# isl-org/Open3D-PointNet2-Semantic3D

Measured on AMD Instinct MI355X. Metric: points/sec through SA+FP stack (B=16,N=8192), higher is better.
Workload: dtype f32

## Files before the change

benchlib/accounting.py:

```python
import json
import os

import torch

ROOT = os.path.dirname(os.path.dirname(os.path.abspath(__file__)))

HBM_PEAK_GBS = 8000.0
MFMA_F32_PEAK_TF = 157.3

FPS_KERNELS = ("farthest_point_sample", "fps_gather", "fps_nested")
LATENCY_KERNELS = FPS_KERNELS + ("coarse_geometry", "ball_query_bin")

PMC_FILE = "profiles/r06_pmc_hbm_traffic.json"
PMC_KERNEL_OF = {"fp_mlp_fused_pre": "fp_chain_pipe_kernel", "fp_mlp_fused": "sa_fused_kernel<2", "sa_mlp_max_fused": "sa_fused_kernel<3, 1, 1, 2"}


def pmc_traffic(kernel):
    try:
        with open(os.path.join(ROOT, PMC_FILE)) as f:
            ks = json.load(f)["kernels"]
    except (OSError, ValueError, KeyError):
        return None
    key = PMC_KERNEL_OF.get(kernel, kernel)
    hits = [v["traffic_bytes"] for k, v in ks.items() if key in k]
# ... 18 lines not shown
        b, n, m, _, ns = a[:5]
        return "hbm", b * n * 12 + b * m * 12 + b * m * ns * 4 + b * m * 4
    if name == "pn2_ball_query_bin":
        b, n = a[:2]
        return "hbm", b * n * 12 + b * n * 14
    if name == "pn2_group_point":
        b, n, c, m, ns = a[:5]
        return "hbm", b * m * ns * 4 + b * n * c * 4 + b * m * ns * c * 4
    if name == "pn2_sa_group_concat":
        b, n, m, ns, c = a[:5]
        return "hbm", b * m * ns * 4 + b * n * (3 + c) * 4 + b * m * 12 + b * m * ns * (3 + c) * 4
    if name == "pn2_three_nn":
        b, n, m = a[:3]
        return "hbm", b * n * 12 + b * m * 12 + b * n * 24
    if name == "pn2_three_interpolate":
        b, m, c, n = a[:4]
        return "hbm", b * m * c * 4 + b * n * 24 + b * n * c * 4
    if name == "pn2_fp_interp_concat":
        b, n, m, c1, c2 = a[:5]
        return "hbm", b * m * c2 * 4 + b * n * 24 + b * n * c1 * 4 + b * n * (c1 + c2) * 4
    if name == "pn2_linear":
        rows, cin, cout = a[:3]
        return "mfma", 2 * rows * cin * cout
    if name == "pn2_mlp_chain":
        rows, cin, L = a[0], a[1], a[2]
        widths = a[4:4 + L]
        fl = 0
        for w in widths:
            fl += 2 * rows * cin * w
            cin = w
        return "mfma", fl
    if name == "pn2_mlp_wide":
        rows, cin, L = a[0], a[1], a[3]
        fl = 0
        for w in a[6:6 + L]:
            fl += 2 * rows * cin * w
            cin = w
        return "mfma", fl
    if name == "pn2_sa_mlp_wide":
        b, n, m, ns, c, L = a[:6]
        cin, fl = 3 + c, 0
        for w in a[7:7 + L]:
            fl += 2 * b * m * ns * cin * w
            cin = w
        return "mfma", fl
    if name == "pn2_fp_mlp_wide":
# ... 117 lines not shown
```

include/pn2_abi.h:

```cpp
#ifndef PN2_ABI_H_
#define PN2_ABI_H_

#include <stddef.h>
#include <stdint.h>

#ifdef __cplusplus
extern "C" {
#endif

#define PN2_ABI_VERSION 2

#define PN2_OK 0
#define PN2_EINVAL (-1)
#define PN2_ENULL (-2)
#define PN2_ERANGE (-3)
#define PN2_EUNSUP (-4)

#define PN2_ARITH_STRICT 0
#define PN2_ARITH_FMA 1
#define PN2_ARITH_FMA_ALT 2

int pn2_abi_version(void);
const char *pn2_build_info(void);
const char *pn2_strerror(int code);
// ... 217 lines not shown
                       const double *scene_z_size, const float *label_weights, int num_label_weights, double half_x,
                       double half_y, unsigned long long seed, long long *counter, const int *draw_scene,
                       const int *draw_center, const unsigned char *draw_mask, int mask_cap, const double *draw_rot,
                       void *workspace, size_t workspace_bytes, int *out_info, double *out_finfo, int *out_sel,
                       float *out_data, int *out_labels, float *out_weights, void *stream);

int pn2_scene_ingest_workspace_size(int n, unsigned long long *bytes);
int pn2_scene_ingest(int n, const double *points, const double *colors, const int *labels, double *out_points,
                     float *out_colors, unsigned char *out_labels, int *out_perm, double *out_zrange, long long *out_hist,
                     int *status, void *workspace, size_t workspace_bytes, void *stream);

int pn2_fp_mlp_fused_pre(int b, int n, int m, int c1, const float *dist, const int *idx, const float *points1,
                         const float *z, int nlayers, const int *widths, const float *const *w,
                         const float *const *bias, float *y, void *stream);
int pn2_fp_mlp_fused_pre_ld(int b, int n, int m, int c1, const float *dist, const int *idx, const float *points1,
                            int ld_points1, const float *z, int nlayers, const int *widths, const float *const *w,
                            const float *const *bias, float *y, void *stream);

int pn2_fp_mlp_fused_pre_schedule(int b, int n, int m, int c1, const float *dist, const int *idx, const float *points1,
                                  const float *z, int nlayers, const int *widths, const float *const *w,
                                  const float *const *bias, float *y, int schedule, void *stream);

int pn2_set_sa_row_packing(int on);

int pn2_sa_mlp_fused_pre(int b, int n, int m, int nsample, const float *xyz, const float *new_xyz, const float *zf,
                         const int *idx, int nlayers, const int *widths, const float *const *w,
                         const float *const *bias, int pool, float *out, void *stream);

int pn2_fp_mlp_wide_pre(int b, int n, int m, int c1, const float *dist, const int *idx, const float *points1,
                        const float *z, int nlayers, const int *widths, const float *const *w,
                        const float *const *bias, float *y, void *stream);
int pn2_sa_mlp_wide_pre(int b, int n, int m, int nsample, const float *xyz, const float *new_xyz, const float *zf,
                        const int *idx, int nlayers, const int *widths, const float *const *w,
                        const float *const *bias, int pool, float *y, void *stream);

size_t pn2_ball_query_bin_bytes(int n);
int pn2_ball_query_bin(int b, int n, float radius, const float *xyz1, void *workspace, size_t workspace_bytes, void *stream);
int pn2_ball_query_bin_ld(int b, int n, float radius, const float *xyz1, int ld1, void *workspace, size_t workspace_bytes,
                          void *stream);
int pn2_query_ball_point_binned(int b, int n, int m, float radius, int nsample, const float *xyz1, const float *xyz2,
                                const void *bins, int *idx, int *pts_cnt, int arith_mode, void *stream);

int pn2_group_pool(long long rows, int k, int c, int mode, const float *x, const float *gxyz, float *out, void *stream);
int pn2_group_pool_grad(long long rows, int k, int c, int mode, const float *x, const float *gxyz, const float *dout,
                        float *dx, void *stream);

// ... 225 lines not shown
```

open3d-pointnet2-semantic3d_amd/csrc/pn2_linear.hip:

```cpp
#include <type_traits>

#include "pn2_common.h"
#include "pn2_mfma_stats.h"
#include "pn2_fwd_narrow.h"
#include "pn2_dgrad_wide.h"

namespace {

template <int U, int N, class F>
__device__ __forceinline__ void static_for(F& f) {
    if constexpr (U < N) {
        f(std::integral_constant<int, U>{});
        static_for<U + 1, N>(f);
    }
}

constexpr int kBK = 32;
constexpr int kAS = kBK + 4;

__device__ __forceinline__ void atomic_max_nonneg(float* addr, float v) {
    atomicMax(reinterpret_cast<int*>(addr), __float_as_int(v));
}

template <int WM, int WN, int NT, bool VEC_A, int WK = 1, int ST = 2, bool TB = false, bool XF = false, int GX = 0>
__global__ void __launch_bounds__(256)
linear_kernel(int rows, int cin, int cout, const float* __restrict__ x,
              const float* __restrict__ w, const float* __restrict__ bias, int relu, int pool,
              float* __restrict__ y, double* __restrict__ stats = nullptr, Pn2BnGradEpilogue gepi = Pn2BnGradEpilogue{},
// ... 625 lines not shown
                v = fmaxf(v, __shfl_xor(v, 32));
                v += bb;
                if (relu) v = fmaxf(v, 0.f);
                if (half == 0 && wrow0 < rows) y[(size_t)(wrow0 / 32) * cout + col] = v;
            }
        }
    }
    }
    pn2_bn_finish(fin, gridDim.x * gridDim.y, blockIdx.x + gridDim.x * blockIdx.y);
}

template <int TM, int TN, int G = 2>
int launch_linear_splitk(int rows, int cin, int cout, const float* x, const float* w, const float* bias, int relu,
                         int pool, float* y, hipStream_t st, double* stats = nullptr, const Pn2BnFinish* fin = nullptr) {
    dim3 grid((rows + 32 * TM - 1) / (32 * TM), cout / (32 * TN));
    const bool vec_a = (cin % 4 == 0) && ((uintptr_t)x % 16 == 0);
    const Pn2BnFinish f = fin ? *fin : Pn2BnFinish{};
    if (vec_a) linear_splitk_kernel<TM, TN, true, G><<<grid, 256, 0, st>>>(rows, cin, cout, x, w, bias, relu, pool, y, stats, f);
    else linear_splitk_kernel<TM, TN, false, G><<<grid, 256, 0, st>>>(rows, cin, cout, x, w, bias, relu, pool, y, stats, f);
    PN2_RETURN_IF_LAUNCH_FAILED();
    return PN2_OK;
}

template <int TM, int TN, bool XF = false, int GX = 0, int NWV = 4>
__global__ void __launch_bounds__(64 * NWV, NWV == 4 ? 2 : 1)
linear_wgrad_kernel(int rows, int cin, int cout, int chunk, const float* __restrict__ x,
                    const float* __restrict__ dy, float* __restrict__ dw, Pn2LoadTransform xf = Pn2LoadTransform{},
                    Pn2GradOnLoad gx = Pn2GradOnLoad{}) {
    const int lane = threadIdx.x & 63, half = lane >> 5, l31 = lane & 31;
    const int wave = __builtin_amdgcn_readfirstlane(threadIdx.x >> 6);
    const long long c0 = ((long long)blockIdx.x * NWV + wave) * chunk;
    const int r0 = c0 < rows ? (int)c0 : rows;
    const int r1 = c0 + chunk < rows ? (int)(c0 + chunk) : rows;
    const int m0 = blockIdx.y * 32 * TM, n0 = blockIdx.z * 32 * TN;
    const int hoff = rows > 1 ? half : 0;
    unsigned offa[TM], offb[TN];
#pragma unroll
    for (int t = 0; t < TM; ++t) { const int m = m0 + t * 32 + l31; offa[t] = (unsigned)(hoff * cin + (m < cin ? m : cin - 1)); }
#pragma unroll
    for (int t = 0; t < TN; ++t) { const int n = n0 + t * 32 + l31; offb[t] = (unsigned)(hoff * cout + (n < cout ? n : cout - 1)); }
    float xsc[TM], xsh[TM];
#pragma unroll
    for (int t = 0; t < TM; ++t) {
        const int m = m0 + t * 32 + l31;
        xsc[t] = XF ? xf.scale[m < cin ? m : cin - 1] : 1.f;
        xsh[t] = XF ? xf.shift[m < cin ? m : cin - 1] : 0.f;
// ... 206 lines not shown
    if (cout % 128 == 0 && g_lin_cfg != 0 && g_lin_cfg < 5) {
        if (g_lin_cfg == 1) return PN2_LIN(4, 1, 4, 1);
        if (g_lin_cfg == 2) return PN2_LIN(2, 2, 2, 1);
        if (g_lin_cfg == 3) return PN2_LIN(1, 4, 1, 1);
        return PN2_LIN(1, 2, 1, 2);
    }
    if (cout % 128 == 0) {
        const long long cb = cout / 128;
        const bool vec_a = (cin % 4 == 0) && ((uintptr_t)x % 16 == 0);
        if (((rows + 127) / 128) * cb >= 512 && vec_a && cb > 1) return PN2_LIN(4, 1, 4, 1);
        if (((rows + 63) / 64) * cb >= 512) return PN2_LIN(2, 2, 2, 1);
        if (((rows + 31) / 32) * cb >= 256 || cin < 128) return PN2_LIN(1, 4, 1, 1);
        return PN2_LIN(1, 2, 1, 2);
    }
    if (cout % 64 == 0 && pool <= 1 && rows <= 32768) return PN2_LIN(1, 2, 1, 2);
    if (cout % 64 == 0) return PN2_LIN(4, 1, 2, 1);
    return PN2_LIN(4, 1, 1, 1);
#undef PN2_LIN
}

extern "C" int pn2_linear(int rows, int cin, int cout, const float* x, const float* w,
                          const float* bias, int relu, int pool, float* y, void* stream) {
    return linear_impl(rows, cin, cout, x, w, bias, relu, pool, y, stream, nullptr);
}

extern "C" int pn2_linear_narrow(int rows, int cin, int cout, const float* x, const float* w, const float* bias, float* y,
                                 void* stream) {
    if (rows <= 0 || cin <= 0 || cout <= 0) return PN2_EINVAL;
    if (!x || !w || !y) return PN2_ENULL;
    if (cout > 16 || cin % 4 != 0 || ((uintptr_t)x % 16) != 0 || (size_t)cin * cout * sizeof(float) > 48 * 1024) return PN2_EUNSUP;
    if ((long long)rows + 128 > 0x7fffffffLL) return PN2_ERANGE;
    hipStream_t st = static_cast<hipStream_t>(stream);
    switch (cout) {
#define PN2_NW(N_) case N_: return launch_linear_narrow<N_>(rows, cin, x, w, bias, y, st);
        PN2_NW(1) PN2_NW(2) PN2_NW(3) PN2_NW(4) PN2_NW(5) PN2_NW(6) PN2_NW(7) PN2_NW(8) PN2_NW(9) PN2_NW(10) PN2_NW(11)
        PN2_NW(12) PN2_NW(13) PN2_NW(14) PN2_NW(15) PN2_NW(16)
#undef PN2_NW
    }
    return PN2_EUNSUP;
}

extern "C" int pn2_linear_bn_stats(int rows, int cin, int cout, const float* x, const float* w, float* y,
                                   void* bn_workspace, size_t workspace_bytes, void* stream) {
    if (!bn_workspace) return PN2_ENULL;
    if (!pn2_bn_ws_fits(bn_workspace, workspace_bytes, cout)) return PN2_EINVAL;
    return linear_impl(rows, cin, cout, x, w, nullptr, 0, 0, y, stream, static_cast<double*>(bn_workspace));
// ... 277 lines not shown
```

open3d-pointnet2-semantic3d_amd/csrc/pn2_sa_fused.hip:

```cpp
#include "pn2_common.h"
#include "pn2_layer_stack.h"
#include <atomic>
#include <type_traits>
#include <utility>

namespace {

typedef float f32x4 __attribute__((ext_vector_type(4)));
typedef float f32x16 __attribute__((ext_vector_type(16)));

struct SaFusedParams {
    int n, m, c, groups;
    int kshift;
    int rows;
    int w[3];
    const float* xyz;
    const float* new_xyz;
    const float* points;
    const int* idx;
    const float* dist;
    const float* points1;
    int c1;
    int ldx, ldp, ld1;
    const float* W[3];
// ... 158 lines not shown
        if (kshift == 4) {
            float v0 = acc[nt][0], v1 = acc[nt][8];
#pragma unroll
            for (int r = 1; r < 8; ++r) { v0 = fmaxf(v0, acc[nt][r]); v1 = fmaxf(v1, acc[nt][8 + r]); }
            v0 = fmaxf(v0, __shfl_xor(v0, 32));
            v1 = fmaxf(v1, __shfl_xor(v1, 32));
            if (half == 0) {
                out[(size_t)(2 * g) * wout + nt * 32 + l31] = fmaxf(v0 + bv, 0.f);
                out[(size_t)(2 * g + 1) * wout + nt * 32 + l31] = fmaxf(v1 + bv, 0.f);
            }
        } else {
            float v = acc[nt][0];
#pragma unroll
            for (int r = 1; r < 16; ++r) v = fmaxf(v, acc[nt][r]);
            v = fmaxf(v, __shfl_xor(v, 32));
            v = fmaxf(v + bv, 0.f);
            if (half == 0)
                atomicMax(reinterpret_cast<int*>(out + (size_t)(g >> (kshift - 5)) * wout + nt * 32 + l31), __float_as_int(v));
        }
    }
}

template <int NT>
__device__ __forceinline__ void pool_store_packed(const f32x16 (&acc)[NT], const float* __restrict__ sbias, float* __restrict__ out,
                                                  int wout, int sshift, int nvalid, const int (&gq)[4], int half, int l31) {
#pragma unroll
    for (int nt = 0; nt < NT; ++nt) {
        const float bv = sbias[nt * 32 + l31];
        float v[4];
#pragma unroll
        for (int q = 0; q < 4; ++q)
            v[q] = fmaxf(fmaxf(acc[nt][4 * q], acc[nt][4 * q + 1]), fmaxf(acc[nt][4 * q + 2], acc[nt][4 * q + 3]));
        if (sshift == 3) {
#pragma unroll
            for (int q = 0; q < 4; ++q) {
                const float u = fmaxf(v[q], __shfl_xor(v[q], 32));
                if (half == 0 && q < nvalid) out[(size_t)gq[q] * wout + nt * 32 + l31] = fmaxf(u + bv, 0.f);
            }
        } else if (sshift == 4) {
#pragma unroll
            for (int q = 0; q < 2; ++q) {
                float u = fmaxf(v[2 * q], v[2 * q + 1]);
                u = fmaxf(u, __shfl_xor(u, 32));
                if (half == 0 && q < nvalid) out[(size_t)gq[q] * wout + nt * 32 + l31] = fmaxf(u + bv, 0.f);
            }
        } else {
            float u = fmaxf(fmaxf(v[0], v[1]), fmaxf(v[2], v[3]));
            u = fmaxf(u, __shfl_xor(u, 32));
            if (half == 0) out[(size_t)gq[0] * wout + nt * 32 + l31] = fmaxf(u + bv, 0.f);
        }
    }
}

template <int NT>
__device__ __forceinline__ void rows_store(const f32x16 (&acc)[NT], const float* __restrict__ sbias,
                                           float* __restrict__ obase, int wout, int row0, int rows,
                                           int half, int l31) {
    if (row0 + 32 <= rows) {
        float* __restrict__ o = obase + (size_t)(row0 + 4 * half) * wout + l31;
#pragma unroll
        for (int nt = 0; nt < NT; ++nt) {
            const float bv = sbias[nt * 32 + l31];
#pragma unroll
            for (int r = 0; r < 16; ++r)
                o[((r & 3) + 8 * (r >> 2)) * wout + nt * 32] = fmaxf(acc[nt][r] + bv, 0.f);
        }
        return;
    }
#pragma unroll
    for (int nt = 0; nt < NT; ++nt) {
        const float bv = sbias[nt * 32 + l31];
#pragma unroll
        for (int r = 0; r < 16; ++r) {
            const int row = row0 + acc_chan(r, half);
            if (row < rows) obase[(size_t)row * wout + nt * 32 + l31] = fmaxf(acc[nt][r] + bv, 0.f);
        }
    }
// ... 109 lines not shown
        stage1(sb3, W3, p.bias[2]);
    }
    __syncthreads();
    PN2_CHAIN_STAMP(1);

    constexpr int WOUT = L == 1 ? W1 : (L == 2 ? W2 : W3);
    int g_lo = blockIdx.x * NW + wave, g_hi = p.groups, g_step = gridDim.x * NW;
    if ((gridDim.x & 7u) == 0u && (p.groups & 7) == 0) {
        const int per = p.groups >> 3, xcd = blockIdx.x & 7, slot = blockIdx.x >> 3;
        g_lo = xcd * per + slot * NW + wave;
        g_hi = (xcd + 1) * per;
        g_step = (gridDim.x >> 3) * NW;
    }
    int pk_b = 0, pk_nb = 0, pk_bstep = 1, pk_lo = 0, pk_hi = 0;
    if constexpr (PACK) {
        pk_lo = 0; pk_hi = p.groups; pk_b = blockIdx.x; pk_bstep = gridDim.x;
        if ((gridDim.x & 7u) == 0u && (p.groups & 7) == 0) {
            const int per = p.groups >> 3, xcd = blockIdx.x & 7;
            pk_lo = xcd * per; pk_hi = pk_lo + per; pk_b = blockIdx.x >> 3; pk_bstep = gridDim.x >> 3;
        }
        pk_nb = (pk_hi - pk_lo + p.blk - 1) / p.blk;
    }
    for (bool pk_first = true;; pk_b += pk_bstep, pk_first = false) {
    int pk_base = 0, pk_n32 = 0, pk_t16 = 0, pk_n16 = 0, pk_n8 = 0;
    if constexpr (PACK) {
        if (pk_b >= pk_nb) break;
        if (!pk_first) __syncthreads();
        pk_base = pk_lo + pk_b * p.blk;
        const int cnt = min(p.blk, pk_hi - pk_base);
        for (int c0 = 2 * wave; c0 < cnt; c0 += 2 * NW) {
            const int cl = c0 + half;
            const int v = p.idx[(size_t)(pk_base + (cl < cnt ? cl : c0)) * 32 + l31];
            const int first = __shfl(v, lane & 32);
            const unsigned long long diff = __ballot(v != first);
            const unsigned mine = (unsigned)(diff >> (lane & 32));
            const int live = 32 - __clz(mine | 1u);
            if (l31 == 0 && cl < cnt) s_cls[cl] = live <= 8 ? 8 : (live <= 16 ? 16 : 32);
        }
        __syncthreads();
        const int cls = lane < cnt ? s_cls[lane] : 0;
        const unsigned long long m32 = __ballot(cls == 32), m16 = __ballot(cls == 16), m8 = __ballot(cls == 8);
        const int n16 = __popcll(m16), n8 = __popcll(m8);
        const int promote = ((n16 & 1) && (n8 & 3) == 1) ? 1 : 0;
        pk_n32 = __popcll(m32); pk_n16 = n16 + promote; pk_n8 = n8 - promote;
        pk_t16 = (pk_n16 + 1) >> 1;
        if (wave == 0 && lane < cnt) {
            const unsigned long long below = (1ull << lane) - 1ull;
            int tile, slot;
            if (cls == 32) { tile = __popcll(m32 & below); slot = 0; }
            else {
                int c = cls, r = __popcll((cls == 16 ? m16 : m8) & below);
                if (promote && c == 8 && r == n8 - 1) { c = 16; r = n16; }
                if (c == 16) { tile = pk_n32 + (r >> 1); slot = r & 1; }
                else { tile = pk_n32 + pk_t16 + (r >> 2); slot = r & 3; }
            }
            s_desc[tile * 4 + slot] = pk_base + lane;
        }
        __syncthreads();
        g_lo = wave; g_hi = pk_n32 + pk_t16 + ((pk_n8 + 3) >> 2); g_step = NW;
    }
    for (int g = g_lo; g < g_hi; g += g_step, ++tile_no) {
        PN2_CHAIN_STAMP(2);
        size_t prow;
        int pk_sshift = 5, pk_nvalid = 1, pk_gq[4] = {0, 0, 0, 0};
        (void)pk_sshift; (void)pk_nvalid; (void)pk_gq;
        f32x16 a1[NT1];
        zero_acc<NT1>(a1);
        constexpr bool LAST1 = (L == 1);
        const float* w1l = wp1 + half * W1 + l31 * NT1;
        constexpr int S0 = DENSE ? 0 : 2;
        if constexpr (DENSE) {
            const int row = g * 32 + l31;
            prow = (size_t)(row < p.rows ? row : p.rows - 1);
        } else {
            int grp, ii;
            if constexpr (PACK) {
                if (g < pk_n32) { pk_sshift = 5; pk_nvalid = 1; }
                else if (g < pk_n32 + pk_t16) { pk_sshift = 4; pk_nvalid = min(2, pk_n16 - 2 * (g - pk_n32)); }
                else { pk_sshift = 3; pk_nvalid = min(4, pk_n8 - 4 * (g - pk_n32 - pk_t16)); }
#pragma unroll
                for (int q = 0; q < 4; ++q) pk_gq[q] = __builtin_amdgcn_readfirstlane(s_desc[g * 4 + (q < pk_nvalid ? q : 0)]);
                const int q = l31 >> pk_sshift;
                grp = q == 1 ? pk_gq[1] : (q == 2 ? pk_gq[2] : (q == 3 ? pk_gq[3] : pk_gq[0]));
                ii = p.idx[(size_t)grp * 32 + (l31 & ((1 << pk_sshift) - 1))];
            } else {
                grp = (g * 32 + l31) >> p.kshift;
                ii = p.idx[(size_t)g * 32 + l31];
            }
            const int bi = grp / p.m;
            prow = (size_t)bi * p.n + ii;
            const float cxv = p.new_xyz[(size_t)grp * 3 + 0];
            const float cyv = p.new_xyz[(size_t)grp * 3 + 1];
            const float czv = p.new_xyz[(size_t)grp * 3 + 2];
            const float rx = p.xyz[prow * p.ldx + 0] - cxv;
            const float ry = p.xyz[prow * p.ldx + 1] - cyv;
            const float rz = p.xyz[prow * p.ldx + 2] - czv;
            mfma_step<NT1, LAST1>(a1, w1l + 0 * 2 * W1, half ? ry : rx);
            mfma_step<NT1, LAST1>(a1, w1l + 1 * 2 * W1, half ? 0.f : rz);
        }
        if constexpr (INTERP) {
            const float* __restrict__ dr = p.dist + prow * 3;
            const int* __restrict__ ir = p.idx + prow * 3;
            const float d1 = fmaxf(dr[0], 1e-10f), d2 = fmaxf(dr[1], 1e-10f), d3 = fmaxf(dr[2], 1e-10f);
            const float r1 = 1.0f / d1, r2 = 1.0f / d2, r3 = 1.0f / d3;
// ... 407 lines not shown
        p.stats[256 + 2048 + blockIdx.x * NW + wave] = (long long)__builtin_amdgcn_s_memrealtime();
        p.stats[256 + 3072 + blockIdx.x * NW + wave] = t_real0;
    }
    if (p.trace && lane == 0) {
        const int wv = blockIdx.x * NW + wave;
        unsigned long long* cnt = reinterpret_cast<unsigned long long*>(p.trace) + (size_t)p.tag * 1024 + wv;
        const unsigned long long cidx = atomicAdd(cnt, 1ull);
        long long* r = p.trace + 8 * 1024 + (((size_t)p.tag * 1024 + wv) * 16 + (cidx & 15ull)) * 2;
        r[0] = t_real0;
        r[1] = (long long)__builtin_amdgcn_s_memrealtime();
    }
#endif
}

PN2_TUNABLE(int, g_chain_prio, 0)
PN2_TUNABLE(long long*, g_chain_stats, nullptr)
PN2_TUNABLE(int, g_chain_nw, 0)
PN2_TUNABLE(int, g_chain_pipe, 1)
PN2_TUNABLE(int, g_chain_grid, 256)
PN2_TUNABLE(long long*, g_chain_trace, nullptr)
PN2_TUNABLE(int, g_chain_tag, 0)

std::atomic<int> g_sa_row_packing{1};
constexpr size_t kPackLdsBytes = (64 + 64 * 4) * sizeof(int);

template <int L, int NT1, int NT2, int NT3, bool VEC8, bool DENSE, bool POOL, int NW, bool INTERP, bool PREZ>
auto chain_kernel(bool pack, int& err) -> void (*)(SaFusedParams) {
    if constexpr (POOL && !DENSE && !INTERP) {
        if (pack) {
            constexpr auto packed = sa_fused_kernel<L, NT1, NT2, NT3, VEC8, DENSE, POOL, NW, INTERP, PREZ, true>;
            err = pn2_allow_lds<packed>(kPn2CuLdsBytes);
            return packed;
        }
    }
    constexpr auto plain = sa_fused_kernel<L, NT1, NT2, NT3, VEC8, DENSE, POOL, NW, INTERP, PREZ, false>;
    err = pn2_allow_lds<plain>(kPn2CuLdsBytes);
    return plain;
}

inline int pack_block(int groups, int grid) {
    int per = groups, nsl = grid;
    if ((grid & 7) == 0 && (groups & 7) == 0) { per = groups >> 3; nsl = grid >> 3; }
    const int blk = (per + nsl - 1) / nsl;
    return blk < 1 ? 1 : (blk > 64 ? 64 : blk);
}

template <int L, int NT1, int NT2, int NT3, bool VEC8, bool DENSE, bool POOL, bool INTERP = false, bool PREZ = false>
// ... 53 lines not shown
        constexpr bool nw12 = true;
#else
        const bool nw12 = g_chain_nw == 12;
#endif
        if (nw12 && bytes > 78 * 1024 && p.groups >= 2048) {
            constexpr auto kern = sa_fused_kernel<L, NT1, NT2, NT3, VEC8, DENSE, POOL, 12, INTERP, PREZ>;
            if (int e = pn2_allow_lds<kern>(kPn2CuLdsBytes)) return e;
            int grid = g_chain_grid;
            const int need12 = (p.groups + 11) / 12;
            if (grid > need12) grid = need12;
            kern<<<grid, 768, bytes, st>>>(p);
            PN2_RETURN_IF_LAUNCH_FAILED();
            return PN2_OK;
        }
    }
    if (bytes > 78 * 1024 && p.groups >= 2048 && g_chain_nw != 4) {
        int e = 0;
        auto kern = chain_kernel<L, NT1, NT2, NT3, VEC8, DENSE, POOL, 8, INTERP, PREZ>(pack, e);
        if (e) return e;
        int grid = g_chain_grid;
        const int need8 = (p.groups + 7) / 8;
        if (grid > need8) grid = need8;
        p.blk = pack_block(p.groups, grid);
        kern<<<grid, 512, bytes + (pack ? kPackLdsBytes : 0), st>>>(p);
    } else {
        int e = 0;
        auto kern = chain_kernel<L, NT1, NT2, NT3, VEC8, DENSE, POOL, 4, INTERP, PREZ>(pack, e);
        if (e) return e;
        int grid = bytes > 78 * 1024 ? g_chain_grid : g_chain_grid * 2;
        if (grid > need4) grid = need4;
        p.blk = pack_block(p.groups, grid);
        kern<<<grid, 256, bytes + (pack ? kPackLdsBytes : 0), st>>>(p);
    }
    PN2_RETURN_IF_LAUNCH_FAILED();
    return PN2_OK;
}

}

#ifdef PN2_TUNING_HOOKS
extern "C" int pn2_debug_set_chain_stats(long long* dev_ptr) { g_chain_stats = dev_ptr; return 0; }
extern "C" int pn2_debug_set_chain_trace(long long* dev_ptr) { g_chain_trace = dev_ptr; return 0; }
extern "C" int pn2_debug_set_fused(int what, int value) {
    if (what == 6) { g_chain_grid = value; return 0; }
    if (what == 7) { g_chain_nw = value; return 0; }
    if (what == 13) { g_chain_prio = value; return 0; }
    if (what == 14) { g_chain_pipe = value; return 0; }
    if (what == 16) { g_chain_tag = value; return 0; }
    return PN2_EINVAL;
}
#endif

bool pn2_sa_row_packing_enabled() { return g_sa_row_packing.load(std::memory_order_relaxed) != 0; }

extern "C" int pn2_set_sa_row_packing(int on) {
// ... 205 lines not shown
```

open3d-pointnet2-semantic3d_amd/util/pointnet_util.py:

```python

import torch

from . import tf_util
from .._lib import float_array, int_array, launch, lib, ptr, ptr_table, require_cuda, rows_in_place, u64_array
from ..tf_ops import tf_grouping
from ..tf_ops.tf_grouping import query_ball_point_multi, group_point, knn_point, query_ball_point
from ..tf_ops.tf_interpolate import three_interpolate, three_nn
from ..tf_ops.tf_sampling import (farthest_point_sample, farthest_point_sample_and_gather, farthest_point_sample_with_ties,
                                  gather_point, tag_fps_output)

USE_FUSED_SA = True
USE_HOISTED_SA = True
USE_SA_ROW_PACKING = True
_sa_row_packing_told = True
USE_HOISTED_FP = True
USE_FUSED_TRAIN_FRONT = True
USE_MLP_CHAIN = True
USE_MLP_WIDE = True
WIDE_MIN_ROWS = 4096
USE_FUSED_FP = True
_WIDE_WIDTHS = (128, 256, 512)


def sample_and_group(npoint, radius, nsample, xyz, points, knn=False, use_xyz=True, geometry=None):
    plan = None
    if geometry is not None:
        new_xyz, idx = geometry[0], geometry[1]
        plan = geometry[2] if len(geometry) > 2 else None
    else:
        fps_idx, fps_tie, _ = farthest_point_sample_with_ties(npoint, xyz)
        new_xyz = tag_fps_output(gather_point(xyz, fps_idx), fps_tie)
        if knn:
            _, idx = knn_point(nsample, xyz, new_xyz)
        else:
            idx, pts_cnt = query_ball_point(radius, nsample, xyz, new_xyz)
    if USE_FUSED_TRAIN_FRONT and points is not None and use_xyz and points.dtype == torch.float32:
        if points.requires_grad and torch.is_grad_enabled():
# ... 267 lines not shown
        return None
    return _sa_fused_inference(a.xyz, a.new_xyz, a.points, a.idx, a.mlp, a.bn, "conv%d")


def _sa_step_dense_float32(a):
    a.xyz = a.xyz.contiguous()
    a.points = None if a.points is None else a.points.contiguous()
    if a.points is not None and a.points.dtype == torch.bfloat16:
        a.points, a.was_bf16 = a.points.float(), True
    return None


def _sa_route_mlp_max_fused_float32(a):
    return _sa_route_mlp_max_fused(a) if a.was_bf16 else None


def _sa_route_mlp_rows_fused(a):
    mlp = a.mlp
    if not (USE_FUSED_SA and len(mlp) == 3 and mlp[0] == mlp[1] == 128 and mlp[2] % 32 == 0):
        return None
    h = _sa_fused_inference(a.xyz, a.new_xyz, a.points, a.idx, mlp[:2], a.bn, "conv%d", pool=False)
    if h is None:
        return None
    h = tf_util.conv2d(h, mlp[2], [1, 1], padding="VALID", stride=[1, 1], bn=a.bn, is_training=False,
                       scope="conv2", bn_decay=a.bn_decay, pool=a.nsample)
    return h.squeeze(2)


def _sa_wide_layers(a):
    mlp, points = a.mlp, a.points
    if not (USE_MLP_WIDE and USE_FUSED_SA and a.nsample == 32 and points is not None
            and points.dtype == torch.float32 and points.shape[2] % 4 == 0 and 1 <= len(mlp) <= 3
            and all(w in _WIDE_WIDTHS for w in mlp) and a.idx.shape[0] * a.idx.shape[1] * 32 >= WIDE_MIN_ROWS):
        return None
    folded, cprev = [], 3 + points.shape[2]
    for i, cout in enumerate(mlp):
        with tf_util.variable_scope("conv%d" % i):
            if i == 0:
                folded.append(tf_util.folded_dense(cprev, cout, a.bn, (1, 1, cprev, cout), pad_to=32,
                                                   pad_in=-(-cprev // 8) * 8, rotate_rows=cprev - 3))
            else:
                folded.append(tf_util.folded_dense(cprev, cout, a.bn, (1, 1, cprev, cout), pad_to=32))
        cprev = cout
    _sync_sa_row_packing(a.xyz)
    return [f[0] for f in folded], [f[1] for f in folded]


def _sa_route_mlp_wide_pre(a):
# ... 410 lines not shown
```

open3d-pointnet2-semantic3d_amd/util/tf_util.py:

```python
import contextlib
import math
from collections import OrderedDict, namedtuple

import weakref

import torch
import torch.nn.functional as F

from .._lib import BN_WS_FOLDED, BN_WS_SUMMED, BN_WS_UNCLEARED, BN_WS_ZEROED
from .._lib import int_array, launch, layer_arrays, lib, nbytes, ptr, ptr_table, require_cuda, rows_in_place, u64_array

BN_EPSILON = 1e-3


class VariableStore:

    def __init__(self, device="cuda", seed=0):
        self.device = torch.device(device)
        self.params = OrderedDict()
        self.buffers = OrderedDict()
        self._gen = torch.Generator(device="cpu")
        self._gen.manual_seed(seed)
        self._seed = int(seed)
        self._dropout = {}
# ... 166 lines not shown
        if pad_to is not None and cout % pad_to != 0:
            padc = pad_to - cout % pad_to
            w2 = F.pad(w2, (0, padc))
            b2 = F.pad(b2, (0, padc))
        if rotate_rows:
            w2 = torch.cat([w2[cin - rotate_rows:], w2[:cin - rotate_rows]], dim=0)
        if pad_in is not None and pad_in > cin:
            w2 = F.pad(w2, (0, 0, 0, pad_in - cin))
        return w2.contiguous(), b2.contiguous()

    srcs = [w, b] + (list(bnv) if bnv is not None else [])
    return st.folded(key, srcs, make)


def hip_linear(x2d, w, b, relu=True, pool=0):
    require_cuda(x2d, w, b)
    rows, cin = x2d.shape
    cout = w.shape[1]
    x2d = x2d.contiguous()
    orows = rows // pool if pool and pool > 1 else rows
    y = torch.empty((orows, cout), dtype=torch.float32, device=x2d.device)
    launch("pn2_linear", x2d, rows, cin, cout, ptr(x2d), ptr(w), ptr(b), int(bool(relu)), int(pool or 0), ptr(y))
    return y


_SAME = object()


def _launch_stack(name, where, lead, ws, bs, trail, oshape, w0=_SAME, after=()):
    L, widths, wptrs, bptrs = layer_arrays(ws, bs)
    if w0 is not _SAME:
        wptrs = ptr_table([w0] + list(ws[1:]))
    y = torch.empty(oshape, dtype=torch.float32, device=where.device)
    dev = lambda args: [ptr(a) if a is None or isinstance(a, torch.Tensor) else a for a in args]
    ok = launch(name, where, *dev(lead), L, widths, wptrs, bptrs, *dev(trail), ptr(y), *dev(after), may_refuse=True)
    return y if ok else None


def pad_first_layer_rows(w0, cin):
    need = -(-cin // 8) * 8
    return w0 if w0.shape[0] >= need else F.pad(w0, (0, 0, 0, need - w0.shape[0])).contiguous()


def hip_mlp_chain(x2d, ws, bs, pool=0):
    require_cuda(x2d)
    rows, cin = x2d.shape
# ... 907 lines not shown
        return _train_dense(inputs, w2d, b, relu=relu)
    if not (cout <= 1024 and (cout % 4 == 0 or cout <= 256)):
        beta, gamma, mean, var = bnv
        cuts, c0 = [], 0
        while cout - c0 > 256 and (cout - c0) % 4 != 0 or cout - c0 > 1024:
            step = min(1024, (cout - c0) // 4 * 4)
            if (cout - c0 - step) > 256 and step < 1024:
                step = (cout - c0 - 256 + 3) // 4 * 4
            cuts.append((c0, c0 + step))
            c0 += step
        cuts.append((c0, cout))
        outs = [_train_layer(inputs, w2d[:, a:e].contiguous(), None if b is None else b[a:e],
                             (beta[a:e], gamma[a:e], mean[a:e], var[a:e]), bn_decay, relu, pool, defer=False) for a, e in cuts]
        return torch.cat(outs, dim=-1)
    beta, gamma, mean, var = bnv
    decay = 0.9 if bn_decay is None else float(bn_decay)
    z = _TrainDenseBnRelu.apply(inputs.reshape(-1, cin).contiguous(), w2d.contiguous(), b, gamma, beta, mean, var,
                                decay, relu, pool, bool(defer) and not pool and relu and torch.is_grad_enabled())
    return z.reshape(lead + [cout])


def conv2d(inputs, num_output_channels, kernel_size, scope, stride=(1, 1), padding="SAME", data_format="NHWC",
           use_xavier=True, stddev=1e-3, weight_decay=None, activation_fn=torch.relu, bn=False, bn_decay=None,
           is_training=None, pool=0, defer_bn=False):
    if list(kernel_size) != [1, 1] or list(stride) != [1, 1] or data_format != "NHWC":
        raise NotImplementedError("only 1x1 / stride 1 / NHWC conv2d is on the SA/FP path")
    if activation_fn not in (torch.relu, None):
        raise NotImplementedError("activation_fn must be relu or None")
    cin = inputs.shape[-1]
    cout = int(num_output_channels)
    with variable_scope(scope):
        if not is_training:
            w2, b2 = folded_dense(cin, cout, bn, (1, 1, cin, cout), pad_to=32)
            y = hip_linear(inputs.reshape(-1, cin), w2, b2, relu=activation_fn is not None, pool=pool)
            if y.shape[1] != cout:
                y = y[:, :cout]
            lead = list(inputs.shape[:-1])
            if pool and pool > 1:
                lead[-1] //= pool
            return y.reshape(lead + [cout])
        st, w, b, bnv = _dense_variables(cin, cout, bn, (1, 1, cin, cout))
        st.train_epoch += 1
        return _train_layer(inputs, w.reshape(cin, cout), b, bnv, bn_decay, activation_fn is not None, pool,
                            defer=bool(defer_bn) and bn)


def conv1d(inputs, num_output_channels, kernel_size, scope, stride=1, padding="SAME", use_xavier=True,
           stddev=1e-3, weight_decay=None, activation_fn=torch.relu, bn=False, bn_decay=None, is_training=None):
    if kernel_size != 1 or stride != 1:
        raise NotImplementedError("only kernel 1 / stride 1 conv1d is on the SA/FP path")
    cin = inputs.shape[-1]
    cout = int(num_output_channels)
    with variable_scope(scope):
        if not is_training:
            if cout <= 16 and not bn and activation_fn is None:
                st, w, b, _ = _dense_variables(cin, cout, False, (1, cin, cout))
                y = hip_linear_narrow(inputs.reshape(-1, cin), w.detach().reshape(cin, cout), b.detach())
# ... 46 lines not shown
```

Before: 383.3 million.

## Add row-packed pooled linear kernel for SA last layer with duplicate neighbours

Adds a new HIP kernel that runs the final SA conv layer with max-pool, packing groups whose ball-query index lists contain only 8 or 16 distinct leading entries into shared 32-row MFMA tiles. The goal is to skip redundant matmul rows for padded (duplicated) neighbours. The row-classification logic is moved into a shared header and reused by the existing fused SA kernel. The Python path routes to it when nsample is 32, cout is a multiple of 128 and rows exceed a threshold, and falls back to the plain linear kernel if it refuses. This adds a classification pass, data-dependent tile counts and extra LDS use.

```diff
diff --git a/benchlib/accounting.py b/benchlib/accounting.py
--- a/benchlib/accounting.py
+++ b/benchlib/accounting.py
@@ -64,6 +64,9 @@
     if name == "pn2_linear":
         rows, cin, cout = a[:3]
         return "mfma", 2 * rows * cin * cout
+    if name == "pn2_linear_pool_packed":
+        groups, ns, cin, cout = a[:4]
+        return "mfma", 2 * groups * ns * cin * cout
     if name == "pn2_mlp_chain":
         rows, cin, L = a[0], a[1], a[2]
         widths = a[4:4 + L]
diff --git a/include/pn2_abi.h b/include/pn2_abi.h
--- a/include/pn2_abi.h
+++ b/include/pn2_abi.h
@@ -263,6 +263,9 @@
                                   const float *const *bias, float *y, int schedule, void *stream);
 
 int pn2_set_sa_row_packing(int on);
+
+int pn2_linear_pool_packed(int groups, int nsample, int cin, int cout, const float *x, const int *idx, const float *w,
+                           const float *bias, int relu, float *y, void *stream);
 
 int pn2_sa_mlp_fused_pre(int b, int n, int m, int nsample, const float *xyz, const float *new_xyz, const float *zf,
                          const int *idx, int nlayers, const int *widths, const float *const *w,
diff --git a/open3d-pointnet2-semantic3d_amd/csrc/pn2_linear.hip b/open3d-pointnet2-semantic3d_amd/csrc/pn2_linear.hip
--- a/open3d-pointnet2-semantic3d_amd/csrc/pn2_linear.hip
+++ b/open3d-pointnet2-semantic3d_amd/csrc/pn2_linear.hip
@@ -4,6 +4,7 @@
 #include "pn2_mfma_stats.h"
 #include "pn2_fwd_narrow.h"
 #include "pn2_dgrad_wide.h"
+#include "pn2_row_packing.h"
 
 namespace {
 
@@ -675,6 +676,104 @@
     return PN2_OK;
 }
 
+template <int BN, int NTW, int NW>
+__global__ void __launch_bounds__(64 * NW)
+linear_pool_packed_kernel(int groups, int cin, int cout, int blk, const float* __restrict__ x, const int* __restrict__ idx,
+                          const float* __restrict__ w, const float* __restrict__ bias, float* __restrict__ y) {
+    constexpr int BS = BN + 4, NSUB = BN / (32 * NTW), NTH = 64 * NW;
+    extern __shared__ __attribute__((aligned(16))) float pk_lds[];
+    const int tid = threadIdx.x, lane = tid & 63, half = lane >> 5, l31 = lane & 31;
+    const int wave = __builtin_amdgcn_readfirstlane(tid >> 6);
+    const int nkc = (cin + kBK - 1) / kBK;
+    float* Bs = pk_lds;
+    int* s_cls = reinterpret_cast<int*>(Bs + (size_t)nkc * kBK * BS);
+    int* s_desc = s_cls + kPn2PackBlockMax;
+    const int col0 = blockIdx.y * BN;
+    const int base = blockIdx.x * blk;
+    const int cnt = min(blk, groups - base);
+
+    const int nf4 = nkc * kBK * (BN / 4);
+    auto w_load = [&](int e0, f32x4 (&v)[8]) __attribute__((always_inline)) {
+#pragma unroll
+        for (int u = 0; u < 8; ++u) {
+            const int e = e0 + u * NTH + tid;
+            const int k = e / (BN / 4), n4 = e % (BN / 4);
+            const f32x4 t = *reinterpret_cast<const f32x4*>(w + (size_t)(k < cin ? k : cin - 1) * cout + col0 + n4 * 4);
+            v[u] = k < cin ? t : f32x4{0.f, 0.f, 0.f, 0.f};
+        }
+    };
+    auto w_store = [&](int e0, const f32x4 (&v)[8]) __attribute__((always_inline)) {
+#pragma unroll
+        for (int u = 0; u < 8; ++u) {
+            const int e = e0 + u * NTH + tid;
+            if (e < nf4) *reinterpret_cast<f32x4*>(Bs + (e / (BN / 4)) * BS + (e % (BN / 4)) * 4) = v[u];
+        }
+    };
+    f32x4 wv[8];
+    w_load(0, wv);
+    const Pn2PackBlock pk = pn2_pack_classify<NW>(idx, base, cnt, wave, lane, s_cls, s_desc);
+    w_store(0, wv);
+    for (int e0 = NTH * 8; e0 < nf4; e0 += NTH * 8) {
+        w_load(e0, wv);
+        w_store(e0, wv);
+    }
+    __syncthreads();
+
+    const int ntasks = pk.tiles() * NSUB;
+    for (int task = wave; task < ntasks; task += NW) {
+        const int tile = task / NSUB, sub = task % NSUB;
+        int sshift, nvalid, gq[4];
+        pn2_pack_tile(pk, tile, s_desc, sshift, nvalid, gq);
+        const int q = l31 >> sshift;
+        const int grp = q == 1 ? gq[1] : (q == 2 ? gq[2] : (q == 3 ? gq[3] : gq[0]));
+        const float* __restrict__ xr = x + ((size_t)grp * 32 + (l31 & ((1 << sshift) - 1))) * cin + 4 * half;
+        auto fetch = [&](int c, f32x4 (&a)[4]) __attribute__((always_inline)) {
+#pragma unroll
+            for (int t = 0; t < 4; ++t) {
+                const int k = c * kBK + 8 * t + 4 * half;
+                const f32x4 v = *reinterpret_cast<const f32x4*>(xr + (k < cin ? c * kBK + 8 * t : cin - 4 - 4 * half));
+                a[t] = k < cin ? v : f32x4{0.f, 0.f, 0.f, 0.f};
+            }
+        };
+        f32x16 acc[NTW];
+#pragma unroll
+        for (int nt = 0; nt < NTW; ++nt)
+#pragma unroll
+            for (int r = 0; r < 16; ++r) acc[nt][r] = 0.f;
+        const float* bs0 = Bs + (4 * half) * BS + sub * (NTW * 32) + l31;
+        auto b_read = [&](int c, float (&b)[16][NTW]) __attribute__((always_inline)) {
+#pragma unroll
+            for (int s = 0; s < 16; ++s)
+#pragma unroll
+                for (int nt = 0; nt < NTW; ++nt) b[s][nt] = bs0[(c * kBK + 8 * (s >> 2) + (s & 3)) * BS + nt * 32];
+        };
+        f32x4 a_cur[4], a_nxt[4];
+        float b_cur[16][NTW], b_nxt[16][NTW];
+        fetch(0, a_cur);
+        b_read(0, b_cur);
+        for (int c = 0; c < nkc; ++c) {
+            const int cn = c + 1 < nkc ? c + 1 : c;
+            fetch(cn, a_nxt);
+            b_read(cn, b_nxt);
+#pragma unroll
+            for (int t = 0; t < 4; ++t)
+#pragma unroll
+                for (int qq = 0; qq < 4; ++qq)
+#pragma unroll
+                    for (int nt = 0; nt < NTW; ++nt)
+                        acc[nt] = __builtin_amdgcn_mfma_f32_32x32x2f32(a_cur[t][qq], b_cur[4 * t + qq][nt], acc[nt], 0, 0, 0);
+#pragma unroll
+            for (int t = 0; t < 4; ++t) a_cur[t] = a_nxt[t];
+#pragma unroll
+            for (int s = 0; s < 16; ++s)
+#pragma unroll
+                for (int nt = 0; nt < NTW; ++nt) b_cur[s][nt] = b_nxt[s][nt];
+        }
+        const int cofs = col0 + sub * (NTW * 32);
+        pool_store_packed<NTW>(acc, bias + cofs, y + cofs, cout, sshift, nvalid, gq, half, l31);
+    }
+}
+
 template <int TM, int TN, bool XF = false, int GX = 0, int NWV = 4>
 __global__ void __launch_bounds__(64 * NWV, NWV == 4 ? 2 : 1)
 linear_wgrad_kernel(int rows, int cin, int cout, int chunk, const float* __restrict__ x,
@@ -927,6 +1026,29 @@
 extern "C" int pn2_linear(int rows, int cin, int cout, const float* x, const float* w,
                           const float* bias, int relu, int pool, float* y, void* stream) {
     return linear_impl(rows, cin, cout, x, w, bias, relu, pool, y, stream, nullptr);
+}
+
+extern "C" int pn2_linear_pool_packed(int groups, int nsample, int cin, int cout, const float* x, const int* idx, const float* w,
+                                      const float* bias, int relu, float* y, void* stream) {
+    if (groups <= 0 || nsample <= 0 || cin <= 0 || cout <= 0) return PN2_EINVAL;
+    if (!x || !idx || !w || !y) return PN2_ENULL;
+    if (!pn2_sa_row_packing_enabled() || nsample != 32 || !relu || !bias || cin % 4 != 0 || cout % 128 != 0 ||
+        ((uintptr_t)x % 16) != 0 || ((uintptr_t)w % 16) != 0)
+        return PN2_EUNSUP;
+    if ((long long)groups * 32 + 128 > 0x7fffffffLL) return PN2_ERANGE;
+    const int nkc = (cin + kBK - 1) / kBK;
+    constexpr int kPackedBN = 64;
+    const size_t lds = sizeof(float) * (size_t)nkc * kBK * (kPackedBN + 4) + kPn2PackLdsBytes;
+    if (lds > (size_t)kPn2CuLdsBytes) return PN2_EUNSUP;
+    const int cb = cout / kPackedBN;
+    int blk = (int)(((long long)groups * cb + 255) / 256);
+    blk = blk < 8 ? 8 : (blk > kPn2PackBlockMax ? kPn2PackBlockMax : blk);
+    constexpr auto kern = linear_pool_packed_kernel<kPackedBN, 2, 8>;
+    const int e = pn2_allow_lds<kern>(kPn2CuLdsBytes);
+    if (e) return e;
+    kern<<<dim3((groups + blk - 1) / blk, cb), 512, lds, static_cast<hipStream_t>(stream)>>>(groups, cin, cout, blk, x, idx, w, bias, y);
+    PN2_RETURN_IF_LAUNCH_FAILED();
+    return PN2_OK;
 }
 
 extern "C" int pn2_linear_narrow(int rows, int cin, int cout, const float* x, const float* w, const float* bias, float* y,
diff --git a/open3d-pointnet2-semantic3d_amd/csrc/pn2_row_packing.h b/open3d-pointnet2-semantic3d_amd/csrc/pn2_row_packing.h
--- /dev/null
+++ b/open3d-pointnet2-semantic3d_amd/csrc/pn2_row_packing.h
@@ -0,0 +1,93 @@
+#pragma once
+
+#include "pn2_common.h"
+
+namespace {
+
+typedef float f32x16 __attribute__((ext_vector_type(16)));
+
+constexpr int kPn2PackBlockMax = 64;
+constexpr size_t kPn2PackLdsBytes = (kPn2PackBlockMax + kPn2PackBlockMax * 4) * sizeof(int);
+
+struct Pn2PackBlock {
+    int n32, t16, n16, n8;
+    __device__ __forceinline__ int tiles() const { return n32 + t16 + ((n8 + 3) >> 2); }
+};
+
+template <int NW>
+__device__ __forceinline__ Pn2PackBlock pn2_pack_classify(const int* __restrict__ idx, int base, int cnt, int wave, int lane,
+                                                          int* s_cls, int* s_desc) {
+    const int half = lane >> 5, l31 = lane & 31;
+    for (int c0 = 2 * wave; c0 < cnt; c0 += 2 * NW) {
+        const int cl = c0 + half;
+        const int v = idx[(size_t)(base + (cl < cnt ? cl : c0)) * 32 + l31];
+        const int first = __shfl(v, lane & 32);
+        const unsigned long long diff = __ballot(v != first);
+        const unsigned mine = (unsigned)(diff >> (lane & 32));
+        const int live = 32 - __clz(mine | 1u);
+        if (l31 == 0 && cl < cnt) s_cls[cl] = live <= 8 ? 8 : (live <= 16 ? 16 : 32);
+    }
+    __syncthreads();
+    const int cls = lane < cnt ? s_cls[lane] : 0;
+    const unsigned long long m32 = __ballot(cls == 32), m16 = __ballot(cls == 16), m8 = __ballot(cls == 8);
+    const int n16 = __popcll(m16), n8 = __popcll(m8);
+    const int promote = ((n16 & 1) && (n8 & 3) == 1) ? 1 : 0;
+    Pn2PackBlock b;
+    b.n32 = __popcll(m32); b.n16 = n16 + promote; b.n8 = n8 - promote;
+    b.t16 = (b.n16 + 1) >> 1;
+    if (wave == 0 && lane < cnt) {
+        const unsigned long long below = (1ull << lane) - 1ull;
+        int tile, slot;
+        if (cls == 32) { tile = __popcll(m32 & below); slot = 0; }
+        else {
+            int c = cls, r = __popcll((cls == 16 ? m16 : m8) & below);
+            if (promote && c == 8 && r == n8 - 1) { c = 16; r = n16; }
+            if (c == 16) { tile = b.n32 + (r >> 1); slot = r & 1; }
+            else { tile = b.n32 + b.t16 + (r >> 2); slot = r & 3; }
+        }
+        s_desc[tile * 4 + slot] = base + lane;
+    }
+    __syncthreads();
+    return b;
+}
+
+__device__ __forceinline__ void pn2_pack_tile(const Pn2PackBlock& b, int g, const int* s_desc, int& sshift, int& nvalid, int (&gq)[4]) {
+    if (g < b.n32) { sshift = 5; nvalid = 1; }
+    else if (g < b.n32 + b.t16) { sshift = 4; nvalid = min(2, b.n16 - 2 * (g - b.n32)); }
+    else { sshift = 3; nvalid = min(4, b.n8 - 4 * (g - b.n32 - b.t16)); }
+#pragma unroll
+    for (int q = 0; q < 4; ++q) gq[q] = __builtin_amdgcn_readfirstlane(s_desc[g * 4 + (q < nvalid ? q : 0)]);
+}
+
+template <int NT>
+__device__ __forceinline__ void pool_store_packed(const f32x16 (&acc)[NT], const float* __restrict__ sbias, float* __restrict__ out,
+                                                  int wout, int sshift, int nvalid, const int (&gq)[4], int half, int l31) {
+#pragma unroll
+    for (int nt = 0; nt < NT; ++nt) {
+        const float bv = sbias[nt * 32 + l31];
+        float v[4];
+#pragma unroll
+        for (int q = 0; q < 4; ++q)
+            v[q] = fmaxf(fmaxf(acc[nt][4 * q], acc[nt][4 * q + 1]), fmaxf(acc[nt][4 * q + 2], acc[nt][4 * q + 3]));
+        if (sshift == 3) {
+#pragma unroll
+            for (int q = 0; q < 4; ++q) {
+                const float u = fmaxf(v[q], __shfl_xor(v[q], 32));
+                if (half == 0 && q < nvalid) out[(size_t)gq[q] * wout + nt * 32 + l31] = fmaxf(u + bv, 0.f);
+            }
+        } else if (sshift == 4) {
+#pragma unroll
+            for (int q = 0; q < 2; ++q) {
+                float u = fmaxf(v[2 * q], v[2 * q + 1]);
+                u = fmaxf(u, __shfl_xor(u, 32));
+                if (half == 0 && q < nvalid) out[(size_t)gq[q] * wout + nt * 32 + l31] = fmaxf(u + bv, 0.f);
+            }
+        } else {
+            float u = fmaxf(fmaxf(v[0], v[1]), fmaxf(v[2], v[3]));
+            u = fmaxf(u, __shfl_xor(u, 32));
+            if (half == 0) out[(size_t)gq[0] * wout + nt * 32 + l31] = fmaxf(u + bv, 0.f);
+        }
+    }
+}
+
+}
diff --git a/open3d-pointnet2-semantic3d_amd/csrc/pn2_sa_fused.hip b/open3d-pointnet2-semantic3d_amd/csrc/pn2_sa_fused.hip
--- a/open3d-pointnet2-semantic3d_amd/csrc/pn2_sa_fused.hip
+++ b/open3d-pointnet2-semantic3d_amd/csrc/pn2_sa_fused.hip
@@ -1,5 +1,6 @@
 #include "pn2_common.h"
 #include "pn2_layer_stack.h"
+#include "pn2_row_packing.h"
 #include <atomic>
 #include <type_traits>
 #include <utility>
@@ -204,37 +205,6 @@
 }
 
 template <int NT>
-__device__ __forceinline__ void pool_store_packed(const f32x16 (&acc)[NT], const float* __restrict__ sbias, float* __restrict__ out,
-                                                  int wout, int sshift, int nvalid, const int (&gq)[4], int half, int l31) {
-#pragma unroll
-    for (int nt = 0; nt < NT; ++nt) {
-        const float bv = sbias[nt * 32 + l31];
-        float v[4];
-#pragma unroll
-        for (int q = 0; q < 4; ++q)
-            v[q] = fmaxf(fmaxf(acc[nt][4 * q], acc[nt][4 * q + 1]), fmaxf(acc[nt][4 * q + 2], acc[nt][4 * q + 3]));
-        if (sshift == 3) {
-#pragma unroll
-            for (int q = 0; q < 4; ++q) {
-                const float u = fmaxf(v[q], __shfl_xor(v[q], 32));
-                if (half == 0 && q < nvalid) out[(size_t)gq[q] * wout + nt * 32 + l31] = fmaxf(u + bv, 0.f);
-            }
-        } else if (sshift == 4) {
-#pragma unroll
-            for (int q = 0; q < 2; ++q) {
-                float u = fmaxf(v[2 * q], v[2 * q + 1]);
-                u = fmaxf(u, __shfl_xor(u, 32));
-                if (half == 0 && q < nvalid) out[(size_t)gq[q] * wout + nt * 32 + l31] = fmaxf(u + bv, 0.f);
-            }
-        } else {
-            float u = fmaxf(fmaxf(v[0], v[1]), fmaxf(v[2], v[3]));
-            u = fmaxf(u, __shfl_xor(u, 32));
-            if (half == 0) out[(size_t)gq[0] * wout + nt * 32 + l31] = fmaxf(u + bv, 0.f);
-        }
-    }
-}
-
-template <int NT>
 __device__ __forceinline__ void rows_store(const f32x16 (&acc)[NT], const float* __restrict__ sbias,
                                            float* __restrict__ obase, int wout, int row0, int rows,
                                            int half, int l31) {
@@ -390,42 +360,16 @@
         pk_nb = (pk_hi - pk_lo + p.blk - 1) / p.blk;
     }
     for (bool pk_first = true;; pk_b += pk_bstep, pk_first = false) {
-    int pk_base = 0, pk_n32 = 0, pk_t16 = 0, pk_n16 = 0, pk_n8 = 0;
+    int pk_base = 0;
+    Pn2PackBlock pk = {0, 0, 0, 0};
+    (void)pk;
     if constexpr (PACK) {
         if (pk_b >= pk_nb) break;
         if (!pk_first) __syncthreads();
         pk_base = pk_lo + pk_b * p.blk;
         const int cnt = min(p.blk, pk_hi - pk_base);
-        for (int c0 = 2 * wave; c0 < cnt; c0 += 2 * NW) {
-            const int cl = c0 + half;
-            const int v = p.idx[(size_t)(pk_base + (cl < cnt ? cl : c0)) * 32 + l31];
-            const int first = __shfl(v, lane & 32);
-            const unsigned long long diff = __ballot(v != first);
-            const unsigned mine = (unsigned)(diff >> (lane & 32));
-            const int live = 32 - __clz(mine | 1u);
-            if (l31 == 0 && cl < cnt) s_cls[cl] = live <= 8 ? 8 : (live <= 16 ? 16 : 32);
-        }
-        __syncthreads();
-        const int cls = lane < cnt ? s_cls[lane] : 0;
-        const unsigned long long m32 = __ballot(cls == 32), m16 = __ballot(cls == 16), m8 = __ballot(cls == 8);
-        const int n16 = __popcll(m16), n8 = __popcll(m8);
-        const int promote = ((n16 & 1) && (n8 & 3) == 1) ? 1 : 0;
-        pk_n32 = __popcll(m32); pk_n16 = n16 + promote; pk_n8 = n8 - promote;
-        pk_t16 = (pk_n16 + 1) >> 1;
-        if (wave == 0 && lane < cnt) {
-            const unsigned long long below = (1ull << lane) - 1ull;
-            int tile, slot;
-            if (cls == 32) { tile = __popcll(m32 & below); slot = 0; }
-            else {
-                int c = cls, r = __popcll((cls == 16 ? m16 : m8) & below);
-                if (promote && c == 8 && r == n8 - 1) { c = 16; r = n16; }
-                if (c == 16) { tile = pk_n32 + (r >> 1); slot = r & 1; }
-                else { tile = pk_n32 + pk_t16 + (r >> 2); slot = r & 3; }
-            }
-            s_desc[tile * 4 + slot] = pk_base + lane;
-        }
-        __syncthreads();
-        g_lo = wave; g_hi = pk_n32 + pk_t16 + ((pk_n8 + 3) >> 2); g_step = NW;
+        pk = pn2_pack_classify<NW>(p.idx, pk_base, cnt, wave, lane, s_cls, s_desc);
+        g_lo = wave; g_hi = pk.tiles(); g_step = NW;
     }
     for (int g = g_lo; g < g_hi; g += g_step, ++tile_no) {
         PN2_CHAIN_STAMP(2);
@@ -443,11 +387,7 @@
         } else {
             int grp, ii;
             if constexpr (PACK) {
-                if (g < pk_n32) { pk_sshift = 5; pk_nvalid = 1; }
-                else if (g < pk_n32 + pk_t16) { pk_sshift = 4; pk_nvalid = min(2, pk_n16 - 2 * (g - pk_n32)); }
-                else { pk_sshift = 3; pk_nvalid = min(4, pk_n8 - 4 * (g - pk_n32 - pk_t16)); }
-#pragma unroll
-                for (int q = 0; q < 4; ++q) pk_gq[q] = __builtin_amdgcn_readfirstlane(s_desc[g * 4 + (q < pk_nvalid ? q : 0)]);
+                pn2_pack_tile(pk, g, s_desc, pk_sshift, pk_nvalid, pk_gq);
                 const int q = l31 >> pk_sshift;
                 grp = q == 1 ? pk_gq[1] : (q == 2 ? pk_gq[2] : (q == 3 ? pk_gq[3] : pk_gq[0]));
                 ii = p.idx[(size_t)grp * 32 + (l31 & ((1 << pk_sshift) - 1))];
@@ -901,7 +841,6 @@
 PN2_TUNABLE(int, g_chain_tag, 0)
 
 std::atomic<int> g_sa_row_packing{1};
-constexpr size_t kPackLdsBytes = (64 + 64 * 4) * sizeof(int);
 
 template <int L, int NT1, int NT2, int NT3, bool VEC8, bool DENSE, bool POOL, int NW, bool INTERP, bool PREZ>
 auto chain_kernel(bool pack, int& err) -> void (*)(SaFusedParams) {
@@ -1001,7 +940,7 @@
         const int need8 = (p.groups + 7) / 8;
         if (grid > need8) grid = need8;
         p.blk = pack_block(p.groups, grid);
-        kern<<<grid, 512, bytes + (pack ? kPackLdsBytes : 0), st>>>(p);
+        kern<<<grid, 512, bytes + (pack ? kPn2PackLdsBytes : 0), st>>>(p);
     } else {
         int e = 0;
         auto kern = chain_kernel<L, NT1, NT2, NT3, VEC8, DENSE, POOL, 4, INTERP, PREZ>(pack, e);
@@ -1009,7 +948,7 @@
         int grid = bytes > 78 * 1024 ? g_chain_grid : g_chain_grid * 2;
         if (grid > need4) grid = need4;
         p.blk = pack_block(p.groups, grid);
-        kern<<<grid, 256, bytes + (pack ? kPackLdsBytes : 0), st>>>(p);
+        kern<<<grid, 256, bytes + (pack ? kPn2PackLdsBytes : 0), st>>>(p);
     }
     PN2_RETURN_IF_LAUNCH_FAILED();
     return PN2_OK;
diff --git a/open3d-pointnet2-semantic3d_amd/util/pointnet_util.py b/open3d-pointnet2-semantic3d_amd/util/pointnet_util.py
--- a/open3d-pointnet2-semantic3d_amd/util/pointnet_util.py
+++ b/open3d-pointnet2-semantic3d_amd/util/pointnet_util.py
@@ -13,6 +13,7 @@
 USE_HOISTED_SA = True
 USE_SA_ROW_PACKING = True
 _sa_row_packing_told = True
+POOL_PACKED_MIN_ROWS = 32768
 USE_HOISTED_FP = True
 USE_FUSED_TRAIN_FRONT = True
 USE_MLP_CHAIN = True
@@ -326,8 +327,11 @@
     h = _sa_fused_inference(a.xyz, a.new_xyz, a.points, a.idx, mlp[:2], a.bn, "conv%d", pool=False)
     if h is None:
         return None
+    packed = USE_SA_ROW_PACKING and a.nsample == 32 and mlp[2] % 128 == 0 and h.shape[0] * h.shape[1] * 32 >= POOL_PACKED_MIN_ROWS
+    if packed:
+        _sync_sa_row_packing(a.xyz)
     h = tf_util.conv2d(h, mlp[2], [1, 1], padding="VALID", stride=[1, 1], bn=a.bn, is_training=False,
-                       scope="conv2", bn_decay=a.bn_decay, pool=a.nsample)
+                       scope="conv2", bn_decay=a.bn_decay, pool=a.nsample, pool_idx=a.idx if packed else None)
     return h.squeeze(2)
 
 
diff --git a/open3d-pointnet2-semantic3d_amd/util/tf_util.py b/open3d-pointnet2-semantic3d_amd/util/tf_util.py
--- a/open3d-pointnet2-semantic3d_amd/util/tf_util.py
+++ b/open3d-pointnet2-semantic3d_amd/util/tf_util.py
@@ -212,6 +212,17 @@
     y = torch.empty((orows, cout), dtype=torch.float32, device=x2d.device)
     launch("pn2_linear", x2d, rows, cin, cout, ptr(x2d), ptr(w), ptr(b), int(bool(relu)), int(pool or 0), ptr(y))
     return y
+
+
+def hip_linear_pool_packed(x2d, idx, w, b):
+    require_cuda(x2d, idx, w, b)
+    groups, nsample = idx.shape[0] * idx.shape[1], idx.shape[2]
+    cin, cout = w.shape
+    x2d, idx = x2d.contiguous(), idx.contiguous()
+    y = torch.empty((groups, cout), dtype=torch.float32, device=x2d.device)
+    ok = launch("pn2_linear_pool_packed", x2d, groups, nsample, cin, cout, ptr(x2d), ptr(idx), ptr(w), ptr(b), 1, ptr(y),
+                may_refuse=True)
+    return y if ok else None
 
 
 _SAME = object()
@@ -1165,7 +1176,7 @@
 
 def conv2d(inputs, num_output_channels, kernel_size, scope, stride=(1, 1), padding="SAME", data_format="NHWC",
            use_xavier=True, stddev=1e-3, weight_decay=None, activation_fn=torch.relu, bn=False, bn_decay=None,
-           is_training=None, pool=0, defer_bn=False):
+           is_training=None, pool=0, defer_bn=False, pool_idx=None):
     if list(kernel_size) != [1, 1] or list(stride) != [1, 1] or data_format != "NHWC":
         raise NotImplementedError("only 1x1 / stride 1 / NHWC conv2d is on the SA/FP path")
     if activation_fn not in (torch.relu, None):
@@ -1175,7 +1186,11 @@
     with variable_scope(scope):
         if not is_training:
             w2, b2 = folded_dense(cin, cout, bn, (1, 1, cin, cout), pad_to=32)
-            y = hip_linear(inputs.reshape(-1, cin), w2, b2, relu=activation_fn is not None, pool=pool)
+            y = None
+            if pool_idx is not None and pool == 32 and activation_fn is not None:
+                y = hip_linear_pool_packed(inputs.reshape(-1, cin), pool_idx, w2, b2)
+            if y is None:
+                y = hip_linear(inputs.reshape(-1, cin), w2, b2, relu=activation_fn is not None, pool=pool)
             if y.shape[1] != cout:
                 y = y[:, :cout]
             lead = list(inputs.shape[:-1])
```

Result: faster. 390.8 million, median of 6 (+2.0%).
